# szcompressor/SZ3

Hardware: AMD Instinct MI355X
Metric: compression throughput GB/s + ratio at fixed abs errBound, 512^3 f32 (higher is better)
Workload: dtype f32; 1 GPU; C2: 3D float32 512x512x512 synthetic field per GPU, Lorenzo predictor, abs errBound=0.001, device-resident in -> device-resident Huffman payload; parallelism=slab1, algo=HIP_LORENZO(16), exchange=none (one rank)

## Files before the change

### sz3_amd/csrc/sz3hip_kernels.hip

```cpp
#include <hip/hip_runtime.h>
#include <cstddef>
#include <stdint.h>
#include <type_traits>
#include <mutex>
#include <utility>
#include <vector>
#include "sz3hip_format.h"
#include "sz3hip_kernels.h"

#include "sz3hip_devutil.h"

template <typename T>
__global__ __launch_bounds__(256) void k_minmax(const T *__restrict__ in, uint64_t n, double *partial) {
    double mn = INFINITY, mx = -INFINITY;
    bool has_nan = false;
    for (uint64_t i = (uint64_t)blockIdx.x * blockDim.x + threadIdx.x; i < n; i += (uint64_t)gridDim.x * blockDim.x) {
        double v = (double)in[i];
        if (v < mn) mn = v;
        if (v > mx) mx = v;
        has_nan |= (v != v);
    }
    (void)has_nan;
#pragma unroll
    for (int d = WAVE / 2; d > 0; d >>= 1) {
// ... 3821 lines not shown
    } else {
        for (uint64_t i = tid; i < n_dout * qbytes; i += nth) p.payload[o_dv + i] = ((const uint8_t *)p.dout_val)[i];
    }
    if (predictor == 2 && p.side) {
        const uint64_t nw = side_bytes / 4;
        uint32_t *d = reinterpret_cast<uint32_t *>(p.payload + o_side);
        for (uint64_t i = tid; i < nw; i += nth) d[i] = reinterpret_cast<const uint32_t *>(p.side)[i];
        for (uint64_t i = nw * 4 + tid; i < side_bytes; i += nth) p.payload[o_side + i] = p.side[i];
    }
}
__global__ __launch_bounds__(256) void k_assemble(szk_asm_params p) {
    assemble_body(p, (uint64_t)blockIdx.x * blockDim.x + threadIdx.x, (uint64_t)gridDim.x * blockDim.x);
    assemble_lists(p, (uint64_t)blockIdx.x * blockDim.x + threadIdx.x, (uint64_t)gridDim.x * blockDim.x);
}

#define ROLE_BLOCKS 3u
#define ROLE_SORT_MAX 2048u
struct szk_role_params {
    uint32_t on;
    uint32_t no_book;
    const uint64_t *hist;
    szk_cb_params cb;
    const szk_cb_info *used;
    const uint8_t *used_lens;
    uint32_t *flags;
    int need_seg;
    int exact;
};
__device__ bool book_rejected(const uint64_t *__restrict__ hist, const szk_cb_info *fresh, const uint8_t *__restrict__ fresh_lens,
                              const szk_cb_info *used, const uint8_t *__restrict__ used_lens, bool exact, uint32_t t, uint32_t nt,
                              unsigned long long *s_acc) {
    const uint32_t lo = fresh->sym_min, cnt = fresh->sym_count;
    if (exact) {
        bool diff = used->sym_min != lo || used->sym_count != cnt || used->max_len != fresh->max_len || used->n_symbols != fresh->n_symbols;
        if (!diff)
            for (uint32_t i = t; i < cnt; i += nt) diff |= used_lens[lo + i] != fresh_lens[lo + i];
        if (diff) atomicOr(&s_acc[0], 1ull);
    } else {
        const uint32_t ulo = used->sym_min, ucnt = used->sym_count;
        unsigned long long cu = 0, cf = 0, missing = 0;
        for (uint32_t i = t; i < cnt; i += nt) {
            const unsigned long long h = hist[lo + i];
            if (!h) continue;
            const uint32_t sym = lo + i;
            const uint32_t lu = (sym >= ulo && sym - ulo < ucnt) ? used_lens[sym] : 0u;
            missing |= lu == 0u;
            cu += h * lu;
            cf += h * fresh_lens[sym];
        }
        cu = wave_sum(cu);
        cf = wave_sum(cf);
        const bool miss_any = __ballot(missing != 0) != 0;
        if (lane_id() == 0) {
            if (miss_any) atomicOr(&s_acc[0], 1ull);
            atomicAdd(&s_acc[1], cu);
            atomicAdd(&s_acc[2], cf);
        }
    }
    __syncthreads();
    if (s_acc[0]) return true;
    return !exact && s_acc[1] * 1024ull > s_acc[2] * 1025ull;
}
__device__ void role_book(const szk_role_params &rp, szk_state *state, uint8_t *pool) {
    __shared__ uint32_t s_wtot[CB_THREADS / WAVE];
    __shared__ uint32_t s_over, s_diff;
    __shared__ uint32_t s_first[SZH_MAX_LEN + 2], s_cnt[SZH_MAX_LEN + 2];
    __shared__ uint32_t s_misc[8];
    __shared__ unsigned long long s_total;
    const szk_cb_params &p = rp.cb;
    const uint32_t t = threadIdx.x;
    const uint32_t n_nonzero = p.range[2];
    bool built = false;
    if (n_nonzero > CB_SMALL_SYMS) {
        if (t == 0) *p.mispredict = 1u;
    } else if (n_nonzero == 0) {
        if (t == 0) {
            p.info->n_symbols = 0;
            p.info->max_len = 0;
            p.info->sym_min = 0;
            p.info->sym_count = 0;
            p.info->win_lo = 0;
            p.info->reserved = 0;
        }
        built = true;
    } else {
        uint32_t lo = 0xFFFFu - p.range[0], range = p.range[1] - lo + 1;
        const bool fill = cb_margins(lo, range, n_nonzero);
        if (t < SZH_MAX_LEN + 2) s_cnt[t] = 0;
        if (t == 0) {
            s_over = 0;
            s_total = 0;
            p.info->ts[0] = wall_clock64();
        }
        for (uint32_t i = t; i < range; i += CB_THREADS) {
            p.enc[lo + i] = 0;
            p.lens[lo + i] = 0;
        }
        __syncthreads();
        cb_small<CB_SMALL_SYMS>(rp.hist, p, pool, lo, range, s_wtot, s_over, s_first, s_cnt, s_misc, s_total, fill);
        built = true;
    }
    __shared__ unsigned long long s_acc[3];
    if (t == 0) s_diff = 0;
    if (t < 3) s_acc[t] = 0;
    __syncthreads();
    if (built && book_rejected(rp.hist, p.info, p.lens, rp.used, rp.used_lens, rp.exact != 0, t, CB_THREADS, s_acc) && t == 0) s_diff = 1;
    __syncthreads();
    if (t == 0) {
        const uint32_t kind = (s_diff ? 1u : 0u) | (!built ? 2u : 0u) | (rp.need_seg && !rp.flags[1] ? 8u : 0u);
        atomicOr(&state->miss_kind, kind);
        state->mispredict = built ? 0u : 1u;
        state->n_symbols = n_nonzero;
    }
}
__device__ void role_sort(const szk_role_params &rp, const szk_asm_params &ap, bool d, uint8_t *pool) {
    const szk_cb_params &p = rp.cb;
    uint64_t *sk = reinterpret_cast<uint64_t *>(pool);
    uint64_t *idx = d ? p.dout_idx : p.vout_idx;
    void *val = d ? p.dout_val : p.vout_val;
    const bool v32 = d ? p.q_is_32bit != 0 : p.t_is_32bit != 0;
    uint64_t n64 = d ? *p.n_dout : *p.n_vout;
    if (n64 > p.out_cap) n64 = p.out_cap;
    if (n64 > ROLE_SORT_MAX) {
        if (threadIdx.x == 0) atomicOr(&ap.state->miss_kind, 4u);
        return;
    }
    const uint32_t n = (uint32_t)n64;
    if (n == 0) return;
    uint32_t np2 = 2;
    while (np2 < n) np2 <<= 1;
    for (uint32_t i = threadIdx.x; i < np2; i += 256) {
        sk[i] = i < n ? (idx[i] << 16) | i : ~0ull;
    }
    __syncthreads();
    for (uint32_t k = 2; k <= np2; k <<= 1)
        for (uint32_t j = k >> 1; j > 0; j >>= 1) {
            for (uint32_t i = threadIdx.x; i < np2; i += 256) {
                const uint32_t x = i ^ j;
                if (x > i) {
                    const uint64_t a = sk[i], b = sk[x];
                    if ((a > b) == ((i & k) == 0)) {
                        sk[i] = b;
                        sk[x] = a;
                    }
                }
            }
            __syncthreads();
        }
    const uint64_t o_i = d ? ap.state->off.dout_idx : ap.state->off.vout_idx, o_v = d ? ap.state->off.dout_val : ap.state->off.vout_val;
    uint64_t *pi = reinterpret_cast<uint64_t *>(ap.payload + o_i);
    for (uint32_t i = threadIdx.x; i < n; i += 256) {
        const uint64_t k = sk[i];
        const uint32_t from = (uint32_t)(k & 0xFFFFu);
        pi[i] = k >> 16;
        if (v32) reinterpret_cast<uint32_t *>(ap.payload + o_v)[i] = reinterpret_cast<const uint32_t *>(val)[from];
        else reinterpret_cast<uint64_t *>(ap.payload + o_v)[i] = reinterpret_cast<const uint64_t *>(val)[from];
    }
    __syncthreads();
    for (uint32_t i = threadIdx.x; i < n; i += 256) {
        idx[i] = sk[i] >> 16;
        if (v32) reinterpret_cast<uint32_t *>(val)[i] = reinterpret_cast<const uint32_t *>(ap.payload + o_v)[i];
        else reinterpret_cast<uint64_t *>(val)[i] = reinterpret_cast<const uint64_t *>(ap.payload + o_v)[i];
    }
}
template <uint32_t WIN>
__global__ __launch_bounds__(256) void k_pack(const uint16_t *__restrict__ codes, uint64_t n,
                                              const uint32_t *__restrict__ g_enc, const szk_cb_info *__restrict__ info,
                                              const uint16_t *__restrict__ chunk_words,
                                              const uint64_t *__restrict__ group_off, szk_mode mode, uint32_t sym_add,
                                              const szk_state *__restrict__ state, uint8_t *__restrict__ payload, szk_asm_params ap,
                                              uint32_t pack_blocks, szk_role_params rp) {
    constexpr int STAGE_WORDS = SZH_CHUNK_SYMS * SZH_MAX_LEN / 32 + 4;
    __shared__ __align__(16) uint32_t s_enc[WIN];
    __shared__ uint32_t s_enc8[256];
    __shared__ uint8_t s_plen8[256];
    __shared__ __align__(8) uint32_t s_stage[4][STAGE_WORDS];
    if (ap.samp_words && ap.samp_words[SZK_SAMP_READY] && szk_is_narrow(mode)) return;
    const uint32_t roles = rp.on ? ROLE_BLOCKS : 0u;
    if (blockIdx.x < roles) {
        static_assert(WIN * 4 >= ROLE_SORT_MAX * 8 && WIN * 4 >= CB_SMALL_SYMS * 28 + 256, "role scratch fits the table");
        if (blockIdx.x == 0) {
            if (!rp.no_book) role_book(rp, ap.state, reinterpret_cast<uint8_t *>(s_enc));
        } else role_sort(rp, ap, blockIdx.x == 2, reinterpret_cast<uint8_t *>(s_enc));
        return;
    }
    const uint32_t bid = blockIdx.x - roles;
    const uint32_t nblk = gridDim.x - roles;
    if (bid >= pack_blocks) {
        assemble_body(ap, (uint64_t)(bid - pack_blocks) * 256 + threadIdx.x, (uint64_t)(nblk - pack_blocks) * 256);
        if (!ap.lists_by_roles) assemble_lists(ap, (uint64_t)bid * 256 + threadIdx.x, (uint64_t)nblk * 256);
        return;
    }
    const bool narrow = szk_is_narrow(mode);
    if (ap.assumed_narrow && !narrow) return;
    const uint64_t n_full = n / SZH_CHUNK_SYMS, n_chunks = (n + SZH_CHUNK_SYMS - 1) / SZH_CHUNK_SYMS;
    const uint64_t wave_gid = (uint64_t)bid * 4 + threadIdx.x / WAVE, nwaves = (uint64_t)pack_blocks * 4;
    const uint64_t lane_off = (uint64_t)lane_id() * ENC_PER_LANE;
    const int lane = lane_id();
    uint32_t *stage = s_stage[threadIdx.x / WAVE];
    uint32_t *out_base = reinterpret_cast<uint32_t *>(payload + state->off.bitstream);

    auto side = [&](uint64_t ch, uint32_t &before_part, uint64_t &goff) {
        const uint64_t grp = ch / PACK_GROUP;
        const uint32_t cin = (uint32_t)(ch % PACK_GROUP);
        before_part = chunk_words[grp * PACK_GROUP + ((uint32_t)lane < cin ? lane : 0)];
        before_part = (uint32_t)lane < cin ? before_part : 0u;
        goff = group_off[grp];
    };
    CodeRegs cur, nxt;
    uint32_t bp_cur = 0, bp_nxt = 0;
    uint64_t go_cur = 0, go_nxt = 0;
    const uint64_t c_end = n_full, c_step = nwaves;
    uint64_t chunk = wave_gid;
    if (chunk < c_end) {
        fetch_codes(codes, chunk * SZH_CHUNK_SYMS + lane_off, narrow, cur);
        side(chunk, bp_cur, go_cur);
    }
    uint32_t sym_min = info->win_lo;
    const uint32_t sym_count = info->sym_count;
    const bool all_lds = WIN == ENC_WIN && sym_count <= ENC_WIN && info->esc_sym == 0;
    const bool wide = info->max_len > 16;
    if (WIN == ENC_WIN) {
        enc_table_load(s_enc, g_enc, sym_min, sym_count);
    } else {
        const uint32_t centre = sym_min + ENC_WIN / 2;
        sym_min = centre > WIN / 2 ? centre - WIN / 2 : 0u;
        if (sym_min > SZH_HIST_BINS - WIN) sym_min = SZH_HIST_BINS - WIN;
        for (uint32_t i = threadIdx.x; i < WIN; i += 256) s_enc[i] = g_enc[sym_min + i];
    }
    if (narrow) {
        const uint32_t e = g_enc[threadIdx.x != 255u ? threadIdx.x + sym_add : 0u];
        s_enc8[threadIdx.x] = e >> 5;
        s_plen8[threadIdx.x] = (uint8_t)(e & 31u);
    }
    for (int i = lane; i < STAGE_WORDS; i += WAVE) stage[i] = 0;
    __syncthreads();
    for (; chunk < c_end; chunk += c_step) {
        const uint64_t nc = chunk + c_step;
        if (nc < c_end) {
            fetch_codes(codes, nc * SZH_CHUNK_SYMS + lane_off, narrow, nxt);
            side(nc, bp_nxt, go_nxt);
        }
        uint16_t c[ENC_PER_LANE];
        uint32_t nwords;
        if (narrow) {
            const uint32_t wds[4] = {cur.a.x, cur.a.y, cur.a.z, cur.a.w};
#pragma unroll
            for (int i = 0; i < 16; i++) c[i] = (uint16_t)((wds[i >> 2] >> (8 * (i & 3))) & 0xFFu);
            nwords = pack_chunk<4, true>(c, 0, 0, false, s_enc8, g_enc, sym_min, all_lds, stage, s_plen8);
        } else {
            unpack_codes(cur, narrow, sym_add, c);
            nwords = wide ? pack_chunk<2, false, WIN>(c, 0, 0, false, s_enc, g_enc, sym_min, all_lds, stage)
                          : pack_chunk<4, false, WIN>(c, 0, 0, false, s_enc, g_enc, sym_min, all_lds, stage);
        }
        const uint32_t before = wave_sum(bp_cur);
        __builtin_amdgcn_fence(__ATOMIC_RELEASE, "workgroup");
        __builtin_amdgcn_wave_barrier();
        uint32_t *out = out_base + go_cur + before;
        for (uint32_t i = 2 * lane; i < nwords + 2; i += 2 * WAVE) {
            const uint2 wv = *reinterpret_cast<const uint2 *>(&stage[i]);
            *reinterpret_cast<uint2 *>(&stage[i]) = make_uint2(0u, 0u);
#if defined(LAB_PACK) && (LAB_PACK & 4)
            if (wv.x == 0x12345678u && wv.y == 0x9abcdef0u) out[i] = 1;
#else
#ifdef LAB_PACK_NT
            if (i < nwords) __builtin_nontemporal_store(__builtin_bswap32(wv.x), &out[i]);
            if (i + 1 < nwords) __builtin_nontemporal_store(__builtin_bswap32(wv.y), &out[i + 1]);
#else
            if (i < nwords) out[i] = __builtin_bswap32(wv.x);
            if (i + 1 < nwords) out[i + 1] = __builtin_bswap32(wv.y);
#endif
#endif
        }
        __builtin_amdgcn_wave_barrier();
        cur = nxt;
        bp_cur = bp_nxt;
        go_cur = go_nxt;
    }
    if (n_full < n_chunks && wave_gid == 0) {
        const uint64_t base = n_full * SZH_CHUNK_SYMS + lane_off;
        uint16_t c[ENC_PER_LANE];
        load_codes16(codes, base, n, narrow, sym_add, c);
        uint32_t bp;
        uint64_t go;
        side(n_full, bp, go);
        const uint32_t nwords = wide ? pack_chunk<2, false, WIN>(c, base, n, true, s_enc, g_enc, sym_min, all_lds, stage)
                                     : pack_chunk<4, false, WIN>(c, base, n, true, s_enc, g_enc, sym_min, all_lds, stage);
        const uint32_t before = wave_sum(bp);
        __builtin_amdgcn_fence(__ATOMIC_RELEASE, "workgroup");
        __builtin_amdgcn_wave_barrier();
        uint32_t *out = out_base + go + before;
        for (uint32_t i = lane; i < nwords; i += WAVE) out[i] = __builtin_bswap32(stage[i]);
    }
    if (nblk > pack_blocks && !ap.lists_by_roles) assemble_lists(ap, (uint64_t)bid * 256 + threadIdx.x, (uint64_t)nblk * 256);
}

#define PB_THREADS 1024u
#define PB_WAVES (PB_THREADS / WAVE)
#define PB_ASM_BLOCKS 32u
#ifndef PB_PAIR_STRIDE
#define PB_PAIR_STRIDE 133u
#endif
static_assert(PB_PAIR_STRIDE % 2u == 1u && PB_PAIR_STRIDE >= 129u && PB_PAIR_STRIDE <= 255u, "odd, a row holds the 128 window bytes, a byte of the dot product");
__device__ __forceinline__ void packb_emit(uint64_t *stage, uint64_t val, uint32_t len, uint32_t pos) {
    const uint64_t v = val << ((64u - len) & 63u);
    const uint32_t q = pos >> 6, sh = pos & 63u;
    atomicOr(reinterpret_cast<unsigned long long *>(&stage[q]), (unsigned long long)(v >> sh));
    atomicOr(reinterpret_cast<unsigned long long *>(&stage[q + 1]), (unsigned long long)((v << 1) << (63u - sh)));
}
template <typename Flush>
__device__ __forceinline__ uint32_t packb_chunk(const uint4 &cw, const uint32_t *__restrict__ s_pair, const uint32_t *__restrict__ s_enc8,
                                                const uint8_t *__restrict__ s_len8, uint64_t *stage, uint32_t staged, bool &fast_tier, Flush &&flush) {
    const uint32_t w[4] = {cw.x, cw.y, cw.z, cw.w};
    {
        constexpr uint32_t K = 0x40404040u;
        const uint32_t inw = (w[0] + K) & (w[1] + K) & (w[2] + K) & (w[3] + K) & 0x80808080u;
        uint32_t e[8];
#pragma unroll
        for (int k = 0; k < 4; k++) {
            const uint32_t m = w[k] & 0x7F7F7F7Fu;
            const uint32_t a0 = __builtin_amdgcn_udot4(m, PB_PAIR_STRIDE << 8 | 1u, 0u, false) << 2;
            const uint32_t a1 = __builtin_amdgcn_udot4(m, (PB_PAIR_STRIDE << 8 | 1u) << 16, 0u, false) << 2;
            e[2 * k] = *reinterpret_cast<const uint32_t *>(reinterpret_cast<const uint8_t *>(s_pair) + a0);
            e[2 * k + 1] = *reinterpret_cast<const uint32_t *>(reinterpret_cast<const uint8_t *>(s_pair) + a1);
        }
        const uint32_t emin = min(min(min(e[0], e[1]), min(e[2], e[3])), min(min(e[4], e[5]), min(e[6], e[7])));
        uint64_t O[2];
        uint32_t OL[2];
#pragma unroll
        for (int i = 0; i < 2; i++) {
            const uint32_t l0 = e[4 * i] & 31u, l1 = e[4 * i + 1] & 31u, l2 = e[4 * i + 2] & 31u, l3 = e[4 * i + 3] & 31u;
            const uint64_t qa = ((uint64_t)(e[4 * i] >> 5) << l1) | (e[4 * i + 1] >> 5);
            const uint64_t qb = ((uint64_t)(e[4 * i + 2] >> 5) << l3) | (e[4 * i + 3] >> 5);
            const uint32_t lb = l2 + l3;
            OL[i] = l0 + l1 + lb;
            O[i] = (qa << (lb & 63u)) | qb;
        }
        const bool fast = inw == 0x80808080u && emin != 0u && OL[0] <= 64u && OL[1] <= 64u;
        if (!__builtin_amdgcn_ballot_w64(!fast)) {
            const uint32_t bits = OL[0] + OL[1];
            const uint32_t incl = wave_incl_scan(bits);
            const uint32_t total_bits = (uint32_t)__builtin_amdgcn_readlane((int)incl, WAVE - 1);
            const uint32_t pos = 32u * staged + incl - bits;
            packb_emit(stage, O[0], OL[0], pos);
            packb_emit(stage, O[1], OL[1], pos + OL[0]);
            fast_tier = true;
            return (total_bits + 31u) >> 5;
        }
    }
    fast_tier = false;
    flush();
    uint64_t P[8];
    uint32_t PL[8];
#pragma unroll
    for (int k = 0; k < 8; k++) {
        const uint32_t pr = (w[k >> 1] >> (16 * (k & 1))) & 0xFFFFu;
        const uint32_t b0 = pr & 0xFFu, b1 = pr >> 8;
        const uint32_t l1 = s_len8[b1];
        P[k] = ((uint64_t)s_enc8[b0] << l1) | s_enc8[b1];
        PL[k] = (uint32_t)s_len8[b0] + l1;
    }
    uint64_t Q[4];
    uint32_t QL[4];
    bool fit_q = true;
#pragma unroll
    for (int j = 0; j < 4; j++) {
        QL[j] = PL[2 * j] + PL[2 * j + 1];
        Q[j] = (P[2 * j] << (PL[2 * j + 1] & 63u)) | P[2 * j + 1];
        fit_q &= QL[j] <= 64u;
    }
    const bool fit_o = QL[0] + QL[1] <= 64u && QL[2] + QL[3] <= 64u;
    const uint32_t bits = QL[0] + QL[1] + QL[2] + QL[3];
    const uint32_t incl = wave_incl_scan(bits);
    const uint32_t total_bits = (uint32_t)__builtin_amdgcn_readlane((int)incl, WAVE - 1);
    uint32_t pos = incl - bits;
    if (!__builtin_amdgcn_ballot_w64(!fit_o)) {
#pragma unroll
        for (int i = 0; i < 2; i++) {
            const uint32_t len = QL[2 * i] + QL[2 * i + 1];
            if (len) packb_emit(stage, (Q[2 * i] << (QL[2 * i + 1] & 63u)) | Q[2 * i + 1], len, pos);
            pos += len;
        }
    } else if (!__builtin_amdgcn_ballot_w64(!fit_q)) {
#pragma unroll
        for (int j = 0; j < 4; j++) {
            if (QL[j]) packb_emit(stage, Q[j], QL[j], pos);
            pos += QL[j];
        }
    } else {
#pragma unroll
        for (int k = 0; k < 8; k++) {
            if (PL[k]) packb_emit(stage, P[k], PL[k], pos);
            pos += PL[k];
        }
    }
    return (total_bits + 31u) >> 5;
}
#define PB_SCAN_GROUPS 4096u
template <bool SCAN>
__global__ __launch_bounds__(PB_THREADS) void k_pack_b(const uint16_t *__restrict__ codes, uint64_t n, const uint32_t *__restrict__ g_enc,
                                                        const uint16_t *__restrict__ chunk_words, const uint64_t *__restrict__ group_off, szk_mode mode,
                                                        uint32_t sym_add, const szk_state *__restrict__ state, uint8_t *__restrict__ payload,
                                                        szk_asm_params ap, uint32_t pack_blocks, uint32_t split, szk_role_params rp, uint32_t only_sampled,
                                                        const uint32_t *__restrict__ group_sums, uint32_t n_groups, uint64_t *__restrict__ group_off_w,
                                                        uint64_t *__restrict__ total_w) {
    constexpr int STAGE_WORDS = SZH_CHUNK_SYMS * SZH_MAX_LEN / 32 + 4;
    constexpr uint32_t PB_BATCH = 4;
    constexpr int UNIT_STAGE = PB_BATCH * 128 + 8;
    static_assert(2 * UNIT_STAGE >= STAGE_WORDS && UNIT_STAGE % 2 == 0, "the unit's stage also holds one chunk of the slow tiers");
    __shared__ __align__(16) uint32_t s_pair[PB_PAIR_STRIDE * 128];
    __shared__ uint32_t s_enc8[256];
    __shared__ uint8_t s_plen8[256];
    __shared__ __align__(16) uint64_t s_stage[PB_WAVES][UNIT_STAGE];
    __shared__ __align__(16) uint32_t s_goff[SCAN ? PB_SCAN_GROUPS : 4u];
    __shared__ uint32_t s_gw[PB_WAVES];
    __shared__ uint64_t s_total;
    static_assert(sizeof(s_pair) + sizeof(s_enc8) + sizeof(s_plen8) + sizeof(s_stage) + sizeof(s_goff) + sizeof(s_gw) + sizeof(s_total) + 1024 <= 160 * 1024,
                  "k_pack_b's LDS must fit one compute unit");
    auto load_sums = [&]() -> uint4 {
        const uint32_t g0 = 4u * threadIdx.x;
        uint4 q = make_uint4(0u, 0u, 0u, 0u);
        if (g0 < n_groups) q = *reinterpret_cast<const uint4 *>(group_sums + g0);
        q.y = g0 + 1u < n_groups ? q.y : 0u;
        q.z = g0 + 2u < n_groups ? q.z : 0u;
        q.w = g0 + 3u < n_groups ? q.w : 0u;
        return q;
    };
    if ((only_sampled & SZK_PACKB_ONLY_SAMPLED) && !(ap.samp_words && ap.samp_words[SZK_SAMP_READY] && szk_is_narrow(mode))) return;
    const uint32_t roles = rp.on ? ROLE_BLOCKS : 0u;
    if (blockIdx.x < roles) {
        if (threadIdx.x >= 256u) return;
        if (blockIdx.x != 0) role_sort(rp, ap, blockIdx.x == 2, reinterpret_cast<uint8_t *>(s_pair));
        return;
    }
    const uint32_t asm_blocks = gridDim.x - roles - pack_blocks;
    if (blockIdx.x >= roles + pack_blocks) {
        const uint32_t ab = blockIdx.x - roles - pack_blocks;
        if (SCAN && ab == 0) {
            const uint4 q = load_sums();
            const uint32_t ws = wave_sum(q.x + q.y + q.z + q.w);
            if (lane_id() == 0) s_gw[threadIdx.x / WAVE] = ws;
            __syncthreads();
            if (threadIdx.x == 0) {
                uint64_t t = 0;
                for (uint32_t w = 0; w < PB_WAVES; w++) t += s_gw[w];
                s_total = t;
            }
        }
        assemble_body(ap, (uint64_t)ab * PB_THREADS + threadIdx.x, (uint64_t)asm_blocks * PB_THREADS, SCAN ? &s_total : nullptr);
        if (!ap.lists_by_roles) assemble_lists(ap, (uint64_t)ab * PB_THREADS + threadIdx.x, (uint64_t)asm_blocks * PB_THREADS);
        return;
    }
    const uint32_t bid = blockIdx.x - roles;
    if (!szk_is_narrow(mode)) return;
    const uint64_t n_full = n / SZH_CHUNK_SYMS, n_chunks = (n + SZH_CHUNK_SYMS - 1) / SZH_CHUNK_SYMS;
    (void)split;
    const uint32_t wv = (uint32_t)__builtin_amdgcn_readfirstlane((int)(threadIdx.x / WAVE));
    const uint64_t wave_gid = (uint64_t)bid * PB_WAVES + wv, nwaves = (uint64_t)pack_blocks * PB_WAVES;
    const int lane = lane_id();
    const uint8_t *c8 = reinterpret_cast<const uint8_t *>(codes) + (uint64_t)lane * ENC_PER_LANE;
    uint64_t *stage = s_stage[wv];
    uint32_t *out_base = reinterpret_cast<uint32_t *>(payload + state->off.bitstream);
    const uint64_t n_units = (n_full + PB_BATCH - 1) / PB_BATCH;
#ifdef SZ3HIP_LAB
    const bool lab_nost = (only_sampled & SZK_PACKB_LAB_NO_STORES) != 0, lab_nold = (only_sampled & SZK_PACKB_LAB_ONE_UNIT) != 0;
#else
    constexpr bool lab_nost = false, lab_nold = false;
#endif
    struct unit_regs {
        uint4 c[PB_BATCH];
        uint32_t fr;
        uint64_t go;
    };
    auto load_unit_mem = [&](unit_regs &r, uint64_t u) {
        const uint64_t c_lo = u * PB_BATCH, grp = c_lo / PACK_GROUP;
#pragma unroll
        for (uint32_t j = 0; j < PB_BATCH; j++) {
            uint64_t ch = c_lo + j < n_full ? c_lo + j : n_full - 1;
            if (lab_nold) ch %= 4 * nwaves;
            r.c[j] = *reinterpret_cast<const uint4 *>(c8 + ch * SZH_CHUNK_SYMS);
        }
        const uint64_t ci = grp * PACK_GROUP + (uint32_t)lane;
        r.fr = chunk_words[ci < n_chunks ? ci : n_chunks - 1];
        if (!SCAN) r.go = group_off[grp];
    };
    auto load_unit = [&](unit_regs &r, uint64_t u) {
        load_unit_mem(r, u);
        if (SCAN) r.go = s_goff[(u * PB_BATCH) / PACK_GROUP];
    };
    uint32_t *const stage32 = reinterpret_cast<uint32_t *>(stage);
    uint4 *const stage128 = reinterpret_cast<uint4 *>(stage);
    typedef uint32_t u32x4_dw __attribute__((ext_vector_type(4), aligned(4)));
    auto copy_out = [&](uint32_t *out, uint32_t nw) {
        const uint32_t tail = nw & 3u, w_t = (nw & ~3u) + (uint32_t)lane;
        if ((uint32_t)lane < tail) {
            const uint32_t v = stage32[w_t ^ 1u];
            if (!lab_nost || v == 0x12345678u) out[w_t] = __builtin_bswap32(v);
        }
        __builtin_amdgcn_wave_barrier();
#pragma unroll
        for (uint32_t t = 0; t < PB_BATCH; t++) {
            const uint32_t i = t * WAVE + (uint32_t)lane;
            if (4u * i < nw) {
                const uint4 v = stage128[i];
                stage128[i] = make_uint4(0u, 0u, 0u, 0u);
                if (4u * i + 4u <= nw && (!lab_nost || v.x == 0x12345678u)) {
                    u32x4_dw o;
                    o.x = __builtin_bswap32(v.y);
                    o.y = __builtin_bswap32(v.x);
                    o.z = __builtin_bswap32(v.w);
                    o.w = __builtin_bswap32(v.z);
                    *reinterpret_cast<u32x4_dw *>(out + 4u * i) = o;
                }
            }
        }
        __builtin_amdgcn_wave_barrier();
    };
    uint32_t *pend_out = out_base;
    uint32_t pend = 0;
    auto copy_pending = [&]() {
        if (pend) {
            __builtin_amdgcn_fence(__ATOMIC_RELEASE, "workgroup");
            __builtin_amdgcn_wave_barrier();
            copy_out(pend_out, pend);
            pend = 0;
        }
    };
    auto pack_unit = [&](const unit_regs &r, uint64_t unit) {
        const uint64_t c_lo = unit * PB_BATCH;
        const uint32_t first = (uint32_t)(c_lo % PACK_GROUP);
        const uint64_t go = SCAN ? (uint64_t)(uint32_t)__builtin_amdgcn_readfirstlane((int)(uint32_t)r.go) : r.go;
        uint32_t *out = out_base + go + wave_sum((uint32_t)lane < first ? r.fr : 0u);
        __builtin_amdgcn_sched_barrier(0);
        copy_pending();
        uint32_t staged = 0;
        auto flush = [&]() {
            if (staged) {
                __builtin_amdgcn_fence(__ATOMIC_RELEASE, "workgroup");
                __builtin_amdgcn_wave_barrier();
                copy_out(out, staged);
                out += staged;
                staged = 0;
            }
        };
#pragma unroll
        for (uint32_t j = 0; j < PB_BATCH; j++) {
            if (c_lo + j < n_full) {
                bool fast_tier;
                const uint32_t nwords = packb_chunk(r.c[j], s_pair, s_enc8, s_plen8, stage, staged, fast_tier, flush);
                if (fast_tier) {
                    staged += nwords;
                } else {
                    __builtin_amdgcn_fence(__ATOMIC_RELEASE, "workgroup");
                    __builtin_amdgcn_wave_barrier();
                    for (uint32_t i = 2 * lane; i < nwords + 2; i += 2 * WAVE) {
                        const uint64_t v = stage[i >> 1];
                        stage[i >> 1] = 0;
                        if (lab_nost && v != 0x123456789abcdefull) continue;
                        if (i < nwords) out[i] = __builtin_bswap32((uint32_t)(v >> 32));
                        if (i + 1 < nwords) out[i + 1] = __builtin_bswap32((uint32_t)v);
                    }
                    __builtin_amdgcn_wave_barrier();
                    out += nwords;
                }
            }
        }
        pend_out = out;
        pend = staged;
    };
    uint64_t unit = wave_gid;
    unit_regs ra, rb;
    uint4 gq = make_uint4(0u, 0u, 0u, 0u);
    uint32_t g_mine = 0, g_incl = 0;
    if (SCAN) gq = load_sums();
    load_unit_mem(ra, unit < n_units ? unit : n_units - 1);
    if (SCAN) {
        g_mine = gq.x + gq.y + gq.z + gq.w;
        g_incl = wave_incl_scan(g_mine);
        if (lane == WAVE - 1) s_gw[wv] = g_incl;
    }
    if (threadIdx.x < 256u) {
        const uint32_t e = g_enc[threadIdx.x != 255u ? threadIdx.x + sym_add : 0u];
        s_enc8[threadIdx.x] = e >> 5;
        s_plen8[threadIdx.x] = (uint8_t)(e & 31u);
    }
    for (int i = lane; i < UNIT_STAGE; i += WAVE) stage[i] = 0;
    __syncthreads();
    if (SCAN) {
        uint32_t run = g_incl - g_mine;
        for (uint32_t w = 0; w < PB_WAVES; w++) run += w < wv ? s_gw[w] : 0u;
        const uint4 o = make_uint4(run, run + gq.x, run + gq.x + gq.y, run + gq.x + gq.y + gq.z);
        reinterpret_cast<uint4 *>(s_goff)[threadIdx.x] = o;
        if (bid == 0) {
            const uint32_t g0 = 4u * threadIdx.x, ov[4] = {o.x, o.y, o.z, o.w};
#pragma unroll
            for (uint32_t k = 0; k < 4; k++)
                if (g0 + k < n_groups) group_off_w[g0 + k] = ov[k];
            if (threadIdx.x == PB_THREADS - 1u) *total_w = (uint64_t)run + g_mine;
        }
    }
    for (uint32_t i = threadIdx.x; i < PB_PAIR_STRIDE * 128u; i += PB_THREADS) {
        const uint32_t i1 = i / PB_PAIR_STRIDE, i0 = i - i1 * PB_PAIR_STRIDE;
        const uint32_t t0 = i0 < 64u ? i0 + 128u : i0 & 127u, t1 = i1 < 64u ? i1 + 128u : i1;
        const uint32_t l0 = s_plen8[t0], l1 = s_plen8[t1];
        const uint32_t len = l0 + l1;
        s_pair[i] = (i0 < 128u && l0 && l1 && len <= 27u) ? ((((s_enc8[t0] << l1) | s_enc8[t1]) << 5) | len) : 0u;
    }
    __syncthreads();
    if (SCAN) ra.go = s_goff[((unit < n_units ? unit : n_units - 1) * PB_BATCH) / PACK_GROUP];
    while (unit < n_units) {
        uint64_t nu = unit + nwaves;
        load_unit(rb, nu < n_units ? nu : unit);
        __builtin_amdgcn_sched_barrier(0);
        pack_unit(ra, unit);
        unit = nu;
        if (unit >= n_units) break;
        nu = unit + nwaves;
        load_unit(ra, nu < n_units ? nu : unit);
        __builtin_amdgcn_sched_barrier(0);
        pack_unit(rb, unit);
        unit = nu;
    }
    copy_pending();
    if (n_full < n_chunks && wave_gid == 0) {
        const uint64_t base = n_full * SZH_CHUNK_SYMS + (uint64_t)lane * ENC_PER_LANE;
        const uint8_t *cb = reinterpret_cast<const uint8_t *>(codes);
        uint32_t bits = 0;
        uint64_t P[8];
        uint32_t PL[8];
#pragma unroll
        for (int k = 0; k < 8; k++) {
            const uint64_t i0 = base + 2 * k, i1 = i0 + 1;
            const uint32_t b0 = i0 < n ? cb[i0] : 0u, b1 = i1 < n ? cb[i1] : 0u;
            const uint32_t l0 = i0 < n ? s_plen8[b0] : 0u, l1 = i1 < n ? s_plen8[b1] : 0u;
            P[k] = ((uint64_t)(i0 < n ? s_enc8[b0] : 0u) << l1) | (i1 < n ? s_enc8[b1] : 0u);
            PL[k] = l0 + l1;
            bits += PL[k];
        }
        const uint32_t incl = wave_incl_scan(bits);
        const uint32_t total_bits = (uint32_t)__builtin_amdgcn_readlane((int)incl, WAVE - 1);
        uint32_t pos = incl - bits;
#pragma unroll
        for (int k = 0; k < 8; k++) {
            if (PL[k]) packb_emit(stage, P[k], PL[k], pos);
            pos += PL[k];
        }
        const uint32_t nwords = (total_bits + 31u) >> 5;
        const uint64_t grp = n_full / PACK_GROUP;
        const uint32_t cin = (uint32_t)(n_full % PACK_GROUP);
        uint32_t bp = (uint32_t)lane < cin ? chunk_words[grp * PACK_GROUP + lane] : 0u;
        const uint32_t before = wave_sum(bp);
        __builtin_amdgcn_fence(__ATOMIC_RELEASE, "workgroup");
        __builtin_amdgcn_wave_barrier();
        uint32_t *out = out_base + (SCAN ? (uint64_t)s_goff[grp] : group_off[grp]) + before;
        for (uint32_t i = lane; i < nwords; i += WAVE) out[i] = __builtin_bswap32((uint32_t)(stage[i >> 1] >> ((i & 1u) ? 0 : 32)));
    }
}

#ifdef SZ3HIP_LAB
struct szk_merge_params {
    const uint32_t *slots;
    const uint16_t *seg_bits;
    const uint32_t *seg_base;
    const uint32_t *fuse_flag;
};
#define MERGE_BLOCK 16
__global__ __launch_bounds__(256) void k_merge(szk_merge_params mp, uint64_t n, const uint16_t *__restrict__ chunk_words,
                                               const uint64_t *__restrict__ group_off, szk_mode mode, const szk_state *__restrict__ state,
                                               uint8_t *__restrict__ payload, szk_asm_params ap, uint32_t pack_blocks, szk_role_params rp) {
    __shared__ __align__(16) uint32_t s_pool[ENC_WIN];
    const uint32_t roles = rp.on ? ROLE_BLOCKS : 0u;
    if (blockIdx.x < roles) {
        if (blockIdx.x == 0) {
#if defined(LAB_MERGE) && (LAB_MERGE & 1)
            if (threadIdx.x == 0) { ap.state->mispredict = 0; ap.state->n_symbols = rp.cb.range[2]; }
#else
            if (!rp.no_book) role_book(rp, ap.state, reinterpret_cast<uint8_t *>(s_pool));
#endif
            if (threadIdx.x == 0 && *mp.fuse_flag) atomicOr(&ap.state->miss_kind, 64u);
        } else role_sort(rp, ap, blockIdx.x == 2, reinterpret_cast<uint8_t *>(s_pool));
        return;
    }
    const uint32_t bid = blockIdx.x - roles;
    const uint32_t nblk = gridDim.x - roles;
    if (bid >= pack_blocks) {
        assemble_body(ap, (uint64_t)(bid - pack_blocks) * 256 + threadIdx.x, (uint64_t)(nblk - pack_blocks) * 256);
        if (!ap.lists_by_roles) assemble_lists(ap, (uint64_t)bid * 256 + threadIdx.x, (uint64_t)nblk * 256);
        return;
    }
    if (ap.assumed_narrow && !szk_is_narrow(mode)) return;
    const uint64_t n_chunks = (n + SZH_CHUNK_SYMS - 1) / SZH_CHUNK_SYMS, n_segs = n >> 8;
    const uint64_t n_blocks = (n_chunks + MERGE_BLOCK - 1) / MERGE_BLOCK;
    const uint64_t wave_gid = (uint64_t)bid * 4 + threadIdx.x / WAVE, nwaves = (uint64_t)pack_blocks * 4;
    const int lane = lane_id();
    uint32_t *out_base = reinterpret_cast<uint32_t *>(payload + state->off.bitstream);
#if defined(LAB_MERGE) && (LAB_MERGE & 2)
    if (n_blocks) return;
#endif
    for (uint64_t blk = wave_gid; blk < n_blocks; blk += nwaves) {
        const uint64_t chunk0 = blk * MERGE_BLOCK;
        const uint64_t seg = chunk0 * 4 + (uint64_t)lane;
        const bool seg_ok = seg < n_segs;
        const uint32_t sb = seg_ok ? mp.seg_bits[seg] : 0u;
        const uint32_t sa = seg_ok ? mp.seg_base[seg] : 0u;
        const uint64_t grp = chunk0 / PACK_GROUP;
        const uint64_t gc = grp * PACK_GROUP + (uint64_t)(lane & 31);
        const uint32_t cw = (lane < 32 && gc < n_chunks) ? chunk_words[gc] : 0u;
        const uint64_t goff = group_off[grp];
        const uint32_t cw_excl = wave_incl_scan(cw) - cw;
        const uint32_t c_in0 = (uint32_t)(chunk0 % PACK_GROUP);
#pragma unroll 2
        for (uint32_t ci = 0; ci < MERGE_BLOCK; ci++) {
            if (chunk0 + ci >= n_chunks) break;
            const uint32_t nwords = (uint32_t)__builtin_amdgcn_readlane((int)cw, (int)(c_in0 + ci));
            const uint32_t before = (uint32_t)__builtin_amdgcn_readlane((int)cw_excl, (int)(c_in0 + ci));
            uint32_t b[4], base[4];
#pragma unroll
            for (int k = 0; k < 4; k++) {
                b[k] = (uint32_t)__builtin_amdgcn_readlane((int)sb, (int)(4 * ci + k));
                base[k] = (uint32_t)__builtin_amdgcn_readlane((int)sa, (int)(4 * ci + k));
            }
            const uint32_t B1 = b[0], B2 = B1 + b[1], B3 = B2 + b[2];
            uint32_t *out = out_base + goff + before;
            for (uint32_t j0 = (uint32_t)lane; j0 < nwords; j0 += 3 * WAVE) {
                uint32_t w0[3], w1[3], wn[3], rem[3], shv[3];
                bool nxt[3];
#pragma unroll
                for (int u = 0; u < 3; u++) {
                    const uint32_t j = j0 + u * WAVE;
                    const uint32_t bit = (j < nwords ? j : 0u) << 5;
                    const uint32_t k = (bit >= B1) + (bit >= B2) + (bit >= B3);
                    const uint32_t Bk = k == 0 ? 0u : (k == 1 ? B1 : (k == 2 ? B2 : B3));
                    const uint32_t bk = k == 0 ? b[0] : (k == 1 ? b[1] : (k == 2 ? b[2] : b[3]));
                    const uint32_t sk = k == 0 ? base[0] : (k == 1 ? base[1] : (k == 2 ? base[2] : base[3]));
                    const uint32_t sn = k == 0 ? base[1] : (k == 1 ? base[2] : base[3]);
                    const uint32_t bn = k == 0 ? b[1] : (k == 1 ? b[2] : (k == 2 ? b[3] : 0u));
                    const uint32_t o = bit - Bk;
                    shv[u] = o & 31u;
                    rem[u] = bk - o;
                    nxt[u] = rem[u] < 32u && bn != 0u;
                    const uint32_t *src = mp.slots + sk + (o >> 5);
                    w0[u] = src[0];
                    w1[u] = src[1];
                    wn[u] = mp.slots[nxt[u] ? sn : sk];
                }
#pragma unroll
                for (int u = 0; u < 3; u++) {
                    const uint32_t j = j0 + u * WAVE;
                    uint32_t v = (uint32_t)((((uint64_t)w0[u] << 32) | w1[u]) >> (32u - shv[u]));
                    if (rem[u] < 32u) {
                        v &= ~0u << (32u - rem[u]);
                        if (nxt[u]) v |= wn[u] >> rem[u];
                    }
                    if (j < nwords) out[j] = __builtin_bswap32(v);
                }
            }
        }
    }
    if (nblk > pack_blocks && !ap.lists_by_roles) assemble_lists(ap, (uint64_t)bid * 256 + threadIdx.x, (uint64_t)nblk * 256);
}

#endif
__global__ __launch_bounds__(1024) void k_dec_tables(const uint8_t *__restrict__ lens, uint32_t sym_min,
                                                     uint32_t sym_count, szk_dec_tables *t, uint32_t radius, uint32_t esc_sym, uint32_t *zero_word,
                                                     const uint16_t *__restrict__ chunk_words, uint64_t n_chunks, uint64_t *group_off,
                                                     uint64_t *total_words) {
    if (blockIdx.x == 1) {
        scan_groups_body<false>(const_cast<uint16_t *>(chunk_words), n_chunks, group_off, total_words, nullptr, 0, nullptr);
        return;
    }
    if (zero_word && threadIdx.x == 0) *zero_word = 0;
    __shared__ uint32_t s_cnt[SZH_MAX_LEN + 2], s_first_code[SZH_MAX_LEN + 2], s_first_rank[SZH_MAX_LEN + 2];
    __shared__ uint16_t s_tbl[(SZH_MAX_LEN + 1) * 1024];
    const uint32_t tid = threadIdx.x, lane = lane_id();
    if (tid < SZH_MAX_LEN + 2) s_cnt[tid] = 0;
    const uint32_t per = (sym_count + 1023) / 1024;
    const uint32_t q0 = tid * per < sym_count ? tid * per : sym_count, q1 = q0 + per < sym_count ? q0 + per : sym_count;
    for (uint32_t l = 0; l <= SZH_MAX_LEN; l++) s_tbl[l * 1024 + tid] = 0;
    __syncthreads();
    for (uint32_t i = q0; i < q1; i++) {
        const uint32_t l = lens[i];
        if (l && l <= SZH_MAX_LEN) s_tbl[l * 1024 + tid]++;
    }
    __syncthreads();
    for (uint32_t l = 1 + tid / WAVE; l <= SZH_MAX_LEN; l += 1024 / WAVE) {
        uint32_t carry = 0;
        for (uint32_t c0 = 0; c0 < 1024; c0 += WAVE) {
            const uint32_t v = s_tbl[l * 1024 + c0 + lane];
            const uint32_t incl = wave_incl_scan(v);
            s_tbl[l * 1024 + c0 + lane] = (uint16_t)(carry + incl - v);
            carry += __shfl(incl, WAVE - 1, WAVE);
        }
        if (lane == 0) s_cnt[l] = carry;
    }
    __syncthreads();
    if (tid == 0) {
        uint32_t code = 0, rank = 0, maxl = 0;
        for (uint32_t l = 1; l <= SZH_MAX_LEN; l++) {
            code = (code + (l > 1 ? s_cnt[l - 1] : 0)) << (l > 1 ? 1 : 0);
            t->first_code[l] = code;
            t->first_rank[l] = rank;
            t->count[l] = s_cnt[l];
            s_first_code[l] = code;
            s_first_rank[l] = rank;
            rank += s_cnt[l];
            if (s_cnt[l]) maxl = l;
        }
        t->max_len = maxl;
        t->n_coded = rank;
        t->lut_bits = maxl < DEC_LUT_BITS ? maxl : DEC_LUT_BITS;
    }
    __syncthreads();
    for (uint32_t i = q0; i < q1; i++) {
        const uint32_t l = lens[i];
        if (l && l <= SZH_MAX_LEN) t->sorted_syms[s_first_rank[l] + s_tbl[l * 1024 + tid]++] = (uint16_t)(esc_sym && sym_min + i == esc_sym ? 0u : sym_min + i);
    }
    __threadfence();
    __syncthreads();
    uint32_t maxl = 0;
    for (uint32_t l = 1; l <= SZH_MAX_LEN; l++)
        if (s_cnt[l]) maxl = l;
    const uint32_t K = maxl < DEC_LUT_BITS ? maxl : DEC_LUT_BITS;
    for (uint32_t e = tid; e < (1u << K); e += 1024) {
        uint32_t ent = 0;
        for (uint32_t l = 1; l <= K; l++) {
            const uint32_t rel = (e >> (K - l)) - s_first_code[l];
            if (rel < s_cnt[l]) {
                ent = ((uint32_t)t->sorted_syms[s_first_rank[l] + rel] << 8) | l;
                break;
            }
        }
        t->lut[e] = ent;
    }
    if (radius && maxl >= 1 && maxl <= 16) {
        for (uint32_t e = tid; e < (1u << DEC_LUT_BITS); e += 1024) {
            uint32_t used = 0, cnt = 0;
            int d[3] = {0, 0, 0};
            for (int j = 0; j < 3; j++) {
                const uint32_t rem = DEC_LUT_BITS - used;
                const uint32_t w = (e << used) & ((1u << DEC_LUT_BITS) - 1u);
                uint32_t l = 0, sym = 0;
                for (uint32_t q = 1; q <= rem && q <= maxl; q++) {
                    const uint32_t rel = (w >> (DEC_LUT_BITS - q)) - s_first_code[q];
                    if (rel < s_cnt[q]) {
                        l = q;
                        sym = t->sorted_syms[s_first_rank[q] + rel];
                        break;
                    }
                }
                const int delta = (int)sym - (int)radius;
                if (l == 0 || sym == 0 || delta < -127 || delta > 127) break;
                d[cnt++] = delta;
                used += l;
            }
            uint32_t ent = 0;
            if (cnt) {
                const int s2 = cnt >= 2 ? d[0] + d[1] : d[0], d3 = cnt == 3 ? d[2] : 0;
                ent = (used - 1u) | (cnt << 4) | (((uint32_t)d[0] & 0xFFu) << 6) | (((uint32_t)s2 & 0x1FFu) << 14) | (((uint32_t)d3 & 0xFFu) << 23);
            }
            t->mlut[e] = ent;
        }
    }
}

#ifndef DEC_SORTED_LDS
#define DEC_SORTED_LDS 1024u
#endif
#ifndef DEC_STAGE_BYTES
#define DEC_STAGE_BYTES 64u
#endif
template <typename QO>
__device__ __forceinline__ QO dec_dout(const szk_dec_params &p, uint64_t elem) {
    uint64_t lo = 0, hi = p.n_dout;
    while (lo < hi) {
        const uint64_t mid = (lo + hi) >> 1;
        if (p.dout_idx[mid] < elem) lo = mid + 1;
        else hi = mid;
    }
    return lo < p.n_dout && p.dout_idx[lo] == elem ? reinterpret_cast<const QO *>(p.dout_val)[lo] : (QO)0;
}
template <int QB, bool HALF = false, bool MS = false, bool LIST = false>
__global__ __launch_bounds__(256) void k_decode(const uint8_t *__restrict__ payload, szk_dec_params p,
                                                uint16_t *__restrict__ codes) {
    static_assert(!MS || (QB == 4 && HALF), "the multi-symbol form decodes f32 Lorenzo streams into the half-width chain");
    static_assert(!LIST || QB == 0, "the list form writes plain codes");
    using QO = typename std::conditional<QB == 8, int64_t, int32_t>::type;
    if (p.gate && *p.gate == 0) return;
    constexpr uint32_t UNIT = SZH_UNIT_SYMS;
    constexpr uint32_t SORTED_LDS = DEC_SORTED_LDS;
    constexpr uint32_t ELT = QB ? (HALF ? QB / 2 : QB) : 2;
    constexpr uint32_t NP = 16 * ELT / 16;
    constexpr uint32_t NR = NP * 16 >= DEC_STAGE_BYTES ? 1 : DEC_STAGE_BYTES / (NP * 16);
    static_assert((UNIT / 16) % NR == 0, "a unit's rounds are a multiple of the collected rounds");
    __shared__ uint4 s_out[4][64 * (NP * NR + 1)];
    __shared__ uint32_t s_first_code[SZH_MAX_LEN + 2], s_first_rank[SZH_MAX_LEN + 2], s_upper[SZH_MAX_LEN + 2];
    __shared__ uint32_t s_lut[1u << DEC_LUT_BITS];
    __shared__ uint16_t s_sorted[SORTED_LDS];
#ifdef LAB_DEC_PAD
    __shared__ uint32_t s_pad[LAB_DEC_PAD / 4];
    if (p.n == 1) s_pad[threadIdx.x] = 1;
#endif
    const uint32_t max_len = p.tables->max_len, K = p.tables->lut_bits, n_coded = p.tables->n_coded;
    if (threadIdx.x <= SZH_MAX_LEN + 1) {
        const uint32_t l = threadIdx.x;
        const bool in = l >= 1 && l <= SZH_MAX_LEN;
        const uint32_t fc = in ? p.tables->first_code[l] : 0, cnt = in ? p.tables->count[l] : 0;
        s_first_code[l] = fc;
        s_first_rank[l] = in ? p.tables->first_rank[l] : 0;
        s_upper[l] = in && l < max_len ? (fc + cnt) << (32 - l) : 0xFFFFFFFFu;
// ... 1672 lines not shown
```

Before: 2441 GB/s.

## Pack two Huffman chunks per wave scan using left-aligned pair codes

The Huffman pack loop now handles chunks in pairs. It computes both chunks' pair-table octets first, then runs a single wave inclusive scan with the two bit counts packed into the 16-bit halves of one word, instead of two separate scans. The pair lookup table now stores codes left-aligned above the length field, so octet assembly uses alignbit and masks instead of variable 64-bit shifts, and emission skips the left-align shift. This adds control-flow complexity for mixed fast and slow chunks, assumes an even batch size, and assumes per-chunk bit totals fit in 16 bits.

```diff
diff --git a/sz3_amd/csrc/sz3hip_kernels.hip b/sz3_amd/csrc/sz3hip_kernels.hip
--- a/sz3_amd/csrc/sz3hip_kernels.hip
+++ b/sz3_amd/csrc/sz3hip_kernels.hip
@@ -4147,53 +4147,69 @@
 #define PB_PAIR_STRIDE 133u
 #endif
 static_assert(PB_PAIR_STRIDE % 2u == 1u && PB_PAIR_STRIDE >= 129u && PB_PAIR_STRIDE <= 255u, "odd, a row holds the 128 window bytes, a byte of the dot product");
-__device__ __forceinline__ void packb_emit(uint64_t *stage, uint64_t val, uint32_t len, uint32_t pos) {
-    const uint64_t v = val << ((64u - len) & 63u);
-    const uint32_t q = pos >> 6, sh = pos & 63u;
+__device__ __forceinline__ void packb_emit_left(uint64_t *stage, uint64_t v, uint32_t pos) {
+    uint32_t q;
+    asm("v_lshrrev_b32 %0, 6, %1" : "=v"(q) : "v"(pos));
+    const uint32_t sh = pos & 63u;
     atomicOr(reinterpret_cast<unsigned long long *>(&stage[q]), (unsigned long long)(v >> sh));
     atomicOr(reinterpret_cast<unsigned long long *>(&stage[q + 1]), (unsigned long long)((v << 1) << (63u - sh)));
 }
+__device__ __forceinline__ void packb_emit(uint64_t *stage, uint64_t val, uint32_t len, uint32_t pos) {
+    packb_emit_left(stage, val << ((64u - len) & 63u), pos);
+}
+__device__ __forceinline__ uint32_t packb_pair_entry(uint32_t c0, uint32_t l0, uint32_t c1, uint32_t l1) {
+    const uint32_t len = l0 + l1;
+    return (l0 && l1 && len <= 27u) ? ((((c0 << l1) | c1) << (32u - len)) | len) : 0u;
+}
+struct packb_oct {
+    uint64_t O[2];
+    uint32_t OL[2];
+    uint32_t inw;
+    uint32_t emin;
+};
+__device__ __forceinline__ void packb_octets(const uint4 &cw, const uint32_t *__restrict__ s_pair, packb_oct &p) {
+    const uint32_t w[4] = {cw.x, cw.y, cw.z, cw.w};
+    constexpr uint32_t K = 0x40404040u;
+    p.inw = (w[0] + K) & (w[1] + K) & (w[2] + K) & (w[3] + K);
+    uint32_t e[8];
+#pragma unroll
+    for (int k = 0; k < 4; k++) {
+        const uint32_t m = w[k] & 0x7F7F7F7Fu;
+        const uint32_t a0 = __builtin_amdgcn_udot4(m, PB_PAIR_STRIDE << 8 | 1u, 0u, false) << 2;
+        const uint32_t a1 = __builtin_amdgcn_udot4(m, (PB_PAIR_STRIDE << 8 | 1u) << 16, 0u, false) << 2;
+        e[2 * k] = *reinterpret_cast<const uint32_t *>(reinterpret_cast<const uint8_t *>(s_pair) + a0);
+        e[2 * k + 1] = *reinterpret_cast<const uint32_t *>(reinterpret_cast<const uint8_t *>(s_pair) + a1);
+    }
+    p.emin = min(min(min(e[0], e[1]), min(e[2], e[3])), min(min(e[4], e[5]), min(e[6], e[7])));
+#pragma unroll
+    for (int i = 0; i < 2; i++) {
+        const uint32_t e0 = e[4 * i], e1 = e[4 * i + 1], e2 = e[4 * i + 2], e3 = e[4 * i + 3];
+        const uint32_t la = (e0 & 31u) + (e1 & 31u);
+        p.OL[i] = la + (e2 & 31u) + (e3 & 31u);
+        constexpr uint32_t CODE = ~31u;
+        const uint32_t m1 = e1 & CODE, m3 = e3 & CODE;
+        const uint32_t ah = (e0 & CODE) | (m1 >> (e0 & 31u)), al = __builtin_amdgcn_alignbit(m1, 0u, e0);
+        const uint32_t bh = (e2 & CODE) | (m3 >> (e2 & 31u)), bl = __builtin_amdgcn_alignbit(m3, 0u, e2);
+        p.O[i] = ((uint64_t)ah << 32 | al) | (((uint64_t)bh << 32 | bl) >> la);
+    }
+}
+__device__ __forceinline__ uint64_t packb_slow_lanes(const packb_oct &p) {
+    return __builtin_amdgcn_ballot_w64((p.inw & 0x80808080u) != 0x80808080u) | __builtin_amdgcn_ballot_w64(p.emin == 0u) |
+           __builtin_amdgcn_ballot_w64(max(p.OL[0], p.OL[1]) > 64u);
+}
 template <typename Flush>
-__device__ __forceinline__ uint32_t packb_chunk(const uint4 &cw, const uint32_t *__restrict__ s_pair, const uint32_t *__restrict__ s_enc8,
-                                                const uint8_t *__restrict__ s_len8, uint64_t *stage, uint32_t staged, bool &fast_tier, Flush &&flush) {
+__device__ __forceinline__ uint32_t packb_chunk(const uint4 &cw, const uint64_t (&O)[2], const uint32_t (&OL)[2], bool fast, const uint32_t *__restrict__ s_enc8,
+                                                const uint8_t *__restrict__ s_len8, uint64_t *stage, uint32_t staged, Flush &&flush) {
     const uint32_t w[4] = {cw.x, cw.y, cw.z, cw.w};
-    {
-        constexpr uint32_t K = 0x40404040u;
-        const uint32_t inw = (w[0] + K) & (w[1] + K) & (w[2] + K) & (w[3] + K) & 0x80808080u;
-        uint32_t e[8];
-#pragma unroll
-        for (int k = 0; k < 4; k++) {
-            const uint32_t m = w[k] & 0x7F7F7F7Fu;
-            const uint32_t a0 = __builtin_amdgcn_udot4(m, PB_PAIR_STRIDE << 8 | 1u, 0u, false) << 2;
-            const uint32_t a1 = __builtin_amdgcn_udot4(m, (PB_PAIR_STRIDE << 8 | 1u) << 16, 0u, false) << 2;
-            e[2 * k] = *reinterpret_cast<const uint32_t *>(reinterpret_cast<const uint8_t *>(s_pair) + a0);
-            e[2 * k + 1] = *reinterpret_cast<const uint32_t *>(reinterpret_cast<const uint8_t *>(s_pair) + a1);
-        }
-        const uint32_t emin = min(min(min(e[0], e[1]), min(e[2], e[3])), min(min(e[4], e[5]), min(e[6], e[7])));
-        uint64_t O[2];
-        uint32_t OL[2];
-#pragma unroll
-        for (int i = 0; i < 2; i++) {
-            const uint32_t l0 = e[4 * i] & 31u, l1 = e[4 * i + 1] & 31u, l2 = e[4 * i + 2] & 31u, l3 = e[4 * i + 3] & 31u;
-            const uint64_t qa = ((uint64_t)(e[4 * i] >> 5) << l1) | (e[4 * i + 1] >> 5);
-            const uint64_t qb = ((uint64_t)(e[4 * i + 2] >> 5) << l3) | (e[4 * i + 3] >> 5);
-            const uint32_t lb = l2 + l3;
-            OL[i] = l0 + l1 + lb;
-            O[i] = (qa << (lb & 63u)) | qb;
-        }
-        const bool fast = inw == 0x80808080u && emin != 0u && OL[0] <= 64u && OL[1] <= 64u;
-        if (!__builtin_amdgcn_ballot_w64(!fast)) {
-            const uint32_t bits = OL[0] + OL[1];
-            const uint32_t incl = wave_incl_scan(bits);
-            const uint32_t total_bits = (uint32_t)__builtin_amdgcn_readlane((int)incl, WAVE - 1);
-            const uint32_t pos = 32u * staged + incl - bits;
-            packb_emit(stage, O[0], OL[0], pos);
-            packb_emit(stage, O[1], OL[1], pos + OL[0]);
-            fast_tier = true;
-            return (total_bits + 31u) >> 5;
-        }
-    }
-    fast_tier = false;
+    if (fast) {
+        const uint32_t bits = OL[0] + OL[1];
+        const uint32_t incl = wave_incl_scan(bits);
+        const uint32_t total_bits = (uint32_t)__builtin_amdgcn_readlane((int)incl, WAVE - 1);
+        const uint32_t pos = 32u * staged + incl - bits;
+        packb_emit_left(stage, O[0], pos);
+        packb_emit_left(stage, O[1], pos + OL[0]);
+        return (total_bits + 31u) >> 5;
+    }
     flush();
     uint64_t P[8];
     uint32_t PL[8];
@@ -4388,25 +4404,49 @@
                 staged = 0;
             }
         };
-#pragma unroll
-        for (uint32_t j = 0; j < PB_BATCH; j++) {
+        auto one_chunk = [&](const uint4 &cw, const uint64_t (&O)[2], const uint32_t (&OL)[2], bool fast_tier) {
+            const uint32_t nwords = packb_chunk(cw, O, OL, fast_tier, s_enc8, s_plen8, stage, staged, flush);
+            if (fast_tier) {
+                staged += nwords;
+            } else {
+                __builtin_amdgcn_fence(__ATOMIC_RELEASE, "workgroup");
+                __builtin_amdgcn_wave_barrier();
+                for (uint32_t i = 2 * lane; i < nwords + 2; i += 2 * WAVE) {
+                    const uint64_t v = stage[i >> 1];
+                    stage[i >> 1] = 0;
+                    if (lab_nost && v != 0x123456789abcdefull) continue;
+                    if (i < nwords) out[i] = __builtin_bswap32((uint32_t)(v >> 32));
+                    if (i + 1 < nwords) out[i + 1] = __builtin_bswap32((uint32_t)v);
+                }
+                __builtin_amdgcn_wave_barrier();
+                out += nwords;
+            }
+        };
+#pragma unroll
+        for (uint32_t j = 0; j < PB_BATCH; j += 2) {
             if (c_lo + j < n_full) {
-                bool fast_tier;
-                const uint32_t nwords = packb_chunk(r.c[j], s_pair, s_enc8, s_plen8, stage, staged, fast_tier, flush);
-                if (fast_tier) {
-                    staged += nwords;
+                const bool two = c_lo + j + 1 < n_full;
+                packb_oct a, b;
+                packb_octets(r.c[j], s_pair, a);
+                const bool ua = !packb_slow_lanes(a);
+                if (!ua) one_chunk(r.c[j], a.O, a.OL, false);
+                packb_octets(r.c[j + 1], s_pair, b);
+                const bool ub = !packb_slow_lanes(b);
+                if (ua && ub && two) {
+                    const uint32_t bits = (a.OL[0] + a.OL[1]) | ((b.OL[0] + b.OL[1]) << 16);
+                    const uint32_t incl = wave_incl_scan(bits);
+                    const uint32_t totals = (uint32_t)__builtin_amdgcn_readlane((int)incl, WAVE - 1);
+                    const uint32_t excl = incl - bits;
+                    const uint32_t nwa = ((totals & 0xFFFFu) + 31u) >> 5, nwb = ((totals >> 16) + 31u) >> 5;
+                    const uint32_t pa = 32u * staged + (excl & 0xFFFFu), pb = 32u * (staged + nwa) + (excl >> 16);
+                    packb_emit_left(stage, a.O[0], pa);
+                    packb_emit_left(stage, a.O[1], pa + a.OL[0]);
+                    packb_emit_left(stage, b.O[0], pb);
+                    packb_emit_left(stage, b.O[1], pb + b.OL[0]);
+                    staged += nwa + nwb;
                 } else {
-                    __builtin_amdgcn_fence(__ATOMIC_RELEASE, "workgroup");
-                    __builtin_amdgcn_wave_barrier();
-                    for (uint32_t i = 2 * lane; i < nwords + 2; i += 2 * WAVE) {
-                        const uint64_t v = stage[i >> 1];
-                        stage[i >> 1] = 0;
-                        if (lab_nost && v != 0x123456789abcdefull) continue;
-                        if (i < nwords) out[i] = __builtin_bswap32((uint32_t)(v >> 32));
-                        if (i + 1 < nwords) out[i + 1] = __builtin_bswap32((uint32_t)v);
-                    }
-                    __builtin_amdgcn_wave_barrier();
-                    out += nwords;
+                    if (ua) one_chunk(r.c[j], a.O, a.OL, true);
+                    if (two) one_chunk(r.c[j + 1], b.O, b.OL, ub);
                 }
             }
         }
@@ -4448,8 +4488,7 @@
         const uint32_t i1 = i / PB_PAIR_STRIDE, i0 = i - i1 * PB_PAIR_STRIDE;
         const uint32_t t0 = i0 < 64u ? i0 + 128u : i0 & 127u, t1 = i1 < 64u ? i1 + 128u : i1;
         const uint32_t l0 = s_plen8[t0], l1 = s_plen8[t1];
-        const uint32_t len = l0 + l1;
-        s_pair[i] = (i0 < 128u && l0 && l1 && len <= 27u) ? ((((s_enc8[t0] << l1) | s_enc8[t1]) << 5) | len) : 0u;
+        s_pair[i] = i0 < 128u ? packb_pair_entry(s_enc8[t0], l0, s_enc8[t1], l1) : 0u;
     }
     __syncthreads();
     if (SCAN) ra.go = s_goff[((unit < n_units ? unit : n_units - 1) * PB_BATCH) / PACK_GROUP];
```

Result: no change. 2461 GB/s, median of 6 (+0.8%).
